# wwang2/CoarseGrainingVAE

Measured on AMD Instinct MI355X. Metric: train_step_frames_per_sec, higher is better.
Workload: dtype f32

## Files before the change

coarsegrainingvae_amd/_lib.py:

```python
from __future__ import annotations

import ctypes as C
import os
import re
import threading

import torch

from . import ktimer

_PKG = os.path.dirname(os.path.abspath(__file__))
LIB_PATH = os.environ.get("CGV_LIB") or os.path.join(_PKG, "libcgvae_hip.so")
HEADER_PATH = os.path.join(os.path.dirname(_PKG), "include", "cgvae_hip.h")

_lock = threading.Lock()
_lib = None

_p, _i, _f, _sz = C.c_void_p, C.c_int, C.c_float, C.c_size_t

PROTOTYPES = {
    "cgv_version": (_i, []),
    "cgv_last_error_string": (C.c_char_p, []),
    "cgv_timestamp": (_i, [_p, _p]),
    "cgv_timestamp_hz": (_i, []),
    "cgv_sustained_clock_probe": (_i, [_p, _p, _i, _i, _p]),
    "cgv_set_option": (_i, [_i, _i]),
    "cgv_get_option": (_i, [_i]),
    "cgv_reset_options": (_i, []),
    "cgv_rbf_supported": (_i, [_i]),
    "cgv_geom_stride": (_i, [_i]),
    "cgv_geom_unit_offset": (_i, [_i]),
    "cgv_radius_graph_count": (_i, [_p, _p, _i, _i, _f, _i, _p, _p, _p]),
    "cgv_radius_graph_emit": (_i, [_p, _p, _i, _i, _f, _i, _p, _p, _p]),
    "cgv_csr_workspace_bytes": (_sz, [_i]),
    "cgv_csr_build": (_i, [_p, _p, _i, _i, _i, _i, _p, _p, _p, _p, _p, _p, _p, _p, _p, _sz, _p]),
    "cgv_group_plan_workspace_bytes": (_sz, [_i]),
    "cgv_group_plan_build": (_i, [_p, _p, _p, _i, _i, _i, _i, _p, _p, _p, _p, _p, _sz, _p]),
    "cgv_group_plan_radix_workspace_bytes": (_sz, [_i]),
    "cgv_group_plan_build_radix": (_i, [_p, _p, _i, _i, _i, _i, _p, _p, _p, _p, _p, _sz, _p]),
    "cgv_geom_group_stride": (_i, [_i]),
    "cgv_geom_group_unit_offset": (_i, [_i]),
    "cgv_edge_geometry_grouped": (_i, [_p, _p, _p, _p, _p, _i, _i, _f, _p, _p, _p]),
    "cgv_edge_geometry": (_i, [_p, _p, _p, _p, _p, _p, _i, _i, _f, _p, _p, _p]),
    "cgv_plan_jobs_max": (_i, []),
    "cgv_plan_job_bytes": (_i, []),
    "cgv_plan_jobs_build": (_i, [_p, _i, _p]),
    "cgv_geom_jobs_max": (_i, []),
    "cgv_geom_job_bytes": (_i, []),
    "cgv_geom_jobs_build": (_i, [_p, _i, _p]),
    "cgv_segment_reduce": (_i, [_p, _p, _p, _i, _i, _i, _p, _p]),
    "cgv_embedding_rows": (_i, [_p, _p, _i, _i, _i, _i, _p, _p]),
    "cgv_embedding_rows2": (_i, [_p, _p, _i, _i, _i, _p, _p, _p, _i, _i, _i, _p, _i, _p]),
    "cgv_segment_reduce_pair": (_i, [_p, _p, _p, _i, _p, _p, _p, _p, _i, _p, _i, _p]),
    "cgv_segment_broadcast": (_i, [_p, _p, _p, _i, _i, _i, _p, _p]),
    "cgv_equi_msg_fwd": (_i, [_p, _p, _p, _p, _p, _p, _p, _p, _p, _i, _i, _i, _i, C.c_int64, C.c_int64, _p, _p, _p]),
    "cgv_equi_msg_grouped_supported": (_i, [_i, _i, _i]),
    "cgv_equi_msg_fwd_grouped": (_i, [_p] * 9 + [_i, _i, _i, _i, C.c_int64, C.c_int64, _p, _p, _p]),
    "cgv_equi_msg_bwd_workspace_bytes": (_sz, [_i, _i, _i]),
    "cgv_equi_msg_bwd": (_i, [_p] * 13 + [_i, _i, _i, C.c_int64, C.c_int64, _p, _sz, _p]),
    "cgv_pseudo_msg_fwd": (_i, [_p] * 14 + [_i, _i, _i, _i, _p]),
    "cgv_pseudo_msg_fwd_rows": (_i, [_p] * 15 + [_i, _i, _i, _i, C.c_int64, _p]),
    "cgv_pseudo_msg_bwd_workspace_bytes": (_sz, [_i, _i, _i]),
    "cgv_pseudo_msg_bwd": (_i, [_p] * 24 + [_i, _i, _i, _i, C.c_int64, _p, _sz, _p]),
    "cgv_pseudo_msg_bwd_deferred": (_i, [_p] * 22 + [_i, _i, _i, _i, C.c_int64, _p, _sz, _p, _p]),
    "cgv_update_rows_from_vec": (_i, [_p, _p, _i, _i, _p]),
    "cgv_tile_bwd_input_plan": (_i, [_i, _i, _i, _i, _p, _p]),
    "cgv_tile_linear_bwd_input_norm_stack": (_i, [_p, _p, _p, _i, _i, _i, _i, _p, _p, _p, _p, _p, _i, _i, _p]),
    "cgv_update_vec_from_rows": (_i, [_p, _p, _p, _i, _i, _p]),
    "cgv_update_norm_stack_fwd": (_i, [_p, _p, _p, _i, _i, _i, _p]),
# ... 204 lines not shown
    "cgv_cgae_resident_fits": (_i, [_i, _i, _i]),
    "cgv_cgae_workspace_bytes": (_sz, [_i, _i, _i, _i]),
    "cgv_cgae_steps": (_i, [_i] + [_p] * 7 + [_i, _p, C.c_int64, _i, _i, _i, _i, C.c_int64, _i, _f] + [C.c_double] * 4 +
                       [C.c_uint64, _p, _p, _p, _p, _sz, _p]),
    "cgv_cgae_noise": (_i, [C.c_uint64, C.c_int64, _i, _i, _i, _p, _p]),
    "cgv_newman_resident_fits": (_i, [_i, _i]),
    "cgv_newman_groups": (_i, [_i, _i]),
    "cgv_newman_workspace_bytes": (_sz, [_i, _i, _i, _i]),
    "cgv_newman_betweenness": (_i, [_p] * 4 + [_i] * 4 + [_p, _p, _sz, _p]),
    "cgv_newman_components": (_i, [_p] * 5 + [_i] * 4 + [_p, _p, _p, _sz, _p]),
    "cgv_newman_partition": (_i, [_p] * 8 + [_i] * 6 + [_p, _sz, _p]),
    "cgv_baseline_resident_fits": (_i, [_i, _i, _i, _i]),
    "cgv_baseline_workspace_bytes": (_sz, [_i] * 7),
    "cgv_baseline_steps": (_i, [_i, _i, _i] + [_p] * 4 + [_i, _p, C.c_int64] + [_i] * 5 + [_p, _p, _p, _i, C.c_int64, _i, _f] +
                           [C.c_double] * 4 + [_p, _p, _p, _sz, _p]),
    "cgv_baseline_loss_workspace_bytes": (_sz, [_i, _i, _i]),
    "cgv_baseline_loss": (_i, [_p, _p, _p, _i, _i, _i, _f, _p, _p, _p, _sz, _p]),
}


OPTIONS = {"msg_fwd_split": 0, "msg_bwd_split": 1, "csr_build": 2, "pseudo_chunks": 3, "wgrad_tiling": 4, "tile_fwd_lds_min": 5,
           "bwd_input_waves": 6, "pseudo_fwd": 7, "decoder_fat": 8, "decoder_wlds": 9, "skinny_rows": 10, "tile_fwd_bal": 11,
           "optim_one_launch": 12, "decoder_colsplit": 13, "decoder_nodesplit": 14, "bwd_input_split": 15, "msg_bwd_mfma": 16,
           "streamk": 17}


def set_option(name: str, value: int) -> None:
    call("cgv_set_option", OPTIONS[name], int(value))


def get_option(name: str) -> int:
    return int(load().cgv_get_option(OPTIONS[name]))


def reset_options() -> None:
    call("cgv_reset_options")


def header_symbols():
    text = open(HEADER_PATH).read()
    text = re.sub(r"/\*.*?\*/", "", text, flags=re.S)
    return sorted(set(re.findall(r"\b(cgv_[a-z0-9_]+)\s*\(", text)))


def load():
    global _lib
    if _lib is not None:
# ... 80 lines not shown
```

coarsegrainingvae_amd/csrc/api.cpp:

```cpp
#include <stdarg.h>
#include <string.h>
#include <atomic>
#include "cgv_common.h"

namespace cgv {
static thread_local char g_err[512] = "";
void set_error(const char* fmt, ...) {
  va_list ap;
  va_start(ap, fmt);
  vsnprintf(g_err, sizeof(g_err), fmt, ap);
  va_end(ap);
}

static const int g_opt_default[] = {
     -1,    -1,     0,
     0,     0,       448,
     0,   0,         1,
     1,      0,        1,
     0,  2,   1,
     -1,  -1,      0};
static_assert(sizeof(g_opt_default) == CGV_OPT_COUNT * sizeof(int), "one default per CGV_OPT_*");
static std::atomic<int> g_opt[CGV_OPT_COUNT];
static void reset_options() {
  for (int i = 0; i < CGV_OPT_COUNT; ++i) g_opt[i].store(g_opt_default[i], std::memory_order_relaxed);
}
static const bool g_opt_ready = (reset_options(), true);
int option(int id) { return g_opt[id].load(std::memory_order_relaxed); }
}

extern "C" {
int cgv_version(void) { return CGV_VERSION; }
int cgv_set_option(int option, int value) {
  CGV_REQUIRE(option >= 0 && option < CGV_OPT_COUNT, "unknown option");
  cgv::g_opt[option].store(value, std::memory_order_relaxed);
  return 0;
}
int cgv_get_option(int option) {
  if (option < 0 || option >= CGV_OPT_COUNT) return INT32_MIN;
  return cgv::g_opt[option].load(std::memory_order_relaxed);
}
int cgv_reset_options(void) {
  cgv::reset_options();
  return 0;
// ... 16 lines not shown
```

coarsegrainingvae_amd/csrc/batch_plans.hip:

```cpp
#include <cstring>
#include "cgv_common.h"

namespace cgv {

constexpr int PJ_MAX = 8;
struct PlanJob {
  const int64_t* key;
  const int64_t* other;
  const float* ids_f32;
  int* rowptr;
  int* eid;
  int* key_sorted;
  int* other_sorted;
  int* count;
  int* tmp;
  unsigned long long* spill;
  int stride, E, n_rows;
  int edge_begin, row_begin;
  int ids_is_key, pad, pad_to;
  int n_other;
};
struct PlanJobs { int n, total_edges, total_rows, pad; PlanJob job[PJ_MAX]; };

__device__ __forceinline__ int pj_ids(const PlanJob& p, int e) {
  const int t = (int)p.ids_f32[(int64_t)e * p.stride];
  return t == p.pad ? p.pad_to : t;
}
__device__ __forceinline__ int pj_key(const PlanJob& p, int e) {
  if (p.ids_f32 && p.ids_is_key) return pj_ids(p, e);
  return p.key ? (int)p.key[(int64_t)e * p.stride] : e;
}
__device__ __forceinline__ int pj_other(const PlanJob& p, int e) {
  if (p.ids_f32 && !p.ids_is_key) return pj_ids(p, e);
  return p.other ? (int)p.other[(int64_t)e * p.stride] : e;
}

__device__ __forceinline__ int pj_find_edge(const PlanJobs& J, int e) {
  int j = 0;
#pragma unroll
  for (int t = 1; t < PJ_MAX; ++t) if (t < J.n && J.job[t].edge_begin <= e) j = t;
  return j;
}

struct PjRun { int head_lane, len; bool head; };
__device__ __forceinline__ PjRun pj_run(int tag ) {
  const int lane = threadIdx.x & 63;
  const int prev = __shfl_up(tag, 1);
  const bool head = lane == 0 || tag != prev;
  const unsigned long long heads = __ballot(head);
  const unsigned long long below = heads & ((2ull << lane) - 1ull);
  const unsigned long long above = lane == 63 ? 0ull : heads & ~((2ull << lane) - 1ull);
  PjRun r;
  r.head = head;
  r.head_lane = 63 - __clzll((long long)below);
  const int end = above ? __ffsll((long long)above) - 1 : 64;
  r.len = end - r.head_lane;
  return r;
}

__global__ __launch_bounds__(256) void pj_count_k(PlanJobs J) {
  const int e = blockIdx.x * 256 + threadIdx.x;
  const bool active = e < J.total_edges;
  int* addr = nullptr;
  int tag = -1;
  if (active) {
    const int j = pj_find_edge(J, e);
    const PlanJob& p = J.job[j];
    const int r = pj_key(p, e - p.edge_begin);
    addr = p.count + r;
    tag = (j << 27) | r;
  }
  const PjRun run = pj_run(tag);
  if (active && run.head) atomicAdd(addr, run.len);
}

__global__ __launch_bounds__(1024) void pj_scan_k(PlanJobs J) {
  const PlanJob& p = J.job[blockIdx.x];
  const int* in = p.count;
  int* out = p.rowptr;
  const int n = p.n_rows;
  __shared__ int wave_tot[16];
  __shared__ int carry_s;
  const int tid = threadIdx.x, lane = tid & 63, w = tid >> 6;
  if (tid == 0) carry_s = 0;
  __syncthreads();
  for (int base = 0; base < n; base += 1024) {
    const int i = base + tid;
    const int x = (i < n) ? in[i] : 0;
    int incl = x;
    for (int d = 1; d < 64; d <<= 1) {
      const int y = __shfl_up(incl, d);
      if (lane >= d) incl += y;
    }
    if (lane == 63) wave_tot[w] = incl;
    __syncthreads();
    int wave_off = 0;
    for (int k = 0; k < w; ++k) wave_off += wave_tot[k];
// ... 98 lines not shown
  __syncthreads();
  for (int t = tid; t < L; t += 128) {
    const unsigned long long mine = k[t];
    const unsigned partner = (unsigned)(mine >> 32);
    int pos = hist[partner];
    if (hist[partner + 1] - pos > 1)
      for (int u = 0; u < L; ++u) pos += (k[u] >> 32) == partner && k[u] < mine;
    p.eid[beg + pos] = (int)(unsigned)(mine & 0xffffffffull);
    p.other_sorted[beg + pos] = (int)partner;
    p.key_sorted[beg + pos] = r;
  }
}

__global__ __launch_bounds__(128) void pj_row_sort_k(PlanJobs J) {
  __shared__ unsigned long long keys[PJ_LDS_KEYS];
  __shared__ int hist[PJ_HIST_MAX + 1];
  int j = 0;
#pragma unroll
  for (int t = 1; t < PJ_MAX; ++t) if (t < J.n && J.job[t].row_begin <= (int)blockIdx.x) j = t;
  const PlanJob& p = J.job[j];
  const int r = blockIdx.x - p.row_begin;
  const int beg = p.rowptr[r], L = p.rowptr[r + 1] - beg;
  if (L <= 0) return;
  if (L <= PJ_LDS_KEYS && L >= PJ_COUNT_FROM && p.n_other > 0 && p.n_other <= PJ_HIST_MAX) pj_count_row(keys, hist, p, r, beg, L);
  else if (L <= PJ_LDS_KEYS) pj_rank_row(keys, p, r, beg, L);
  else pj_rank_row(p.spill + beg, p, r, beg, L);
}

constexpr int GJ_MAX = 12;
struct GeomJob {
  const float* pos_dst; const float* pos_src;
  const int* dst; const int* src;
  const int2* meta;
  const float* coef;
  float* geom;
  float cutoff;
  int E, R, GS, edge_begin;
};
struct GeomJobs { int n, total_edges; GeomJob job[GJ_MAX]; };

constexpr int GJ_REC_MAX = 28;
__global__ __launch_bounds__(256) void gj_records_k(GeomJobs J) {
  __shared__ __attribute__((aligned(16))) float recs[256][GJ_REC_MAX];
  const int e_first = blockIdx.x * 256;
  const int e_raw = e_first + threadIdx.x;
  const bool valid = e_raw < J.total_edges;
// ... 43 lines not shown
    g[R + 5] = __int_as_float(m.y);
    for (int k = R + 6; k < GS; ++k) g[k] = 0.0f;
  } else {
    const int U = geom_unit_offset(R);
    for (int k = R + 1; k < U; ++k) g[k] = 0.0f;
    g[U + 0] = ux; g[U + 1] = uy; g[U + 2] = uz;
    g[U + 3] = ux; g[U + 4] = uy; g[U + 5] = uz;
    for (int k = U + 6; k < GS; ++k) g[k] = 0.0f;
  }
  if (!one_job) {
    if (valid)
      for (int k4 = 0; k4 < GS / 4; ++k4) dst4[k4] = reinterpret_cast<const float4*>(g)[k4];
    return;
  }
  __syncthreads();
  const int n_rec = min(256, J.total_edges - e_first), GS4 = GS >> 2;
  float4* out4 = reinterpret_cast<float4*>(q.geom + (size_t)(e_first - q.edge_begin) * GS);
  for (int idx = threadIdx.x; idx < n_rec * GS4; idx += 256) {
    const int r = idx / GS4, k4 = idx - r * GS4;
    out4[idx] = reinterpret_cast<const float4*>(recs[r])[k4];
  }
}

__global__ __launch_bounds__(256) void batch_rows_k(const float4* __restrict__ src_a, float4* __restrict__ dst_a,
                                                    float* __restrict__ xyz_a, int n_a, const float4* __restrict__ src_b,
                                                    float4* __restrict__ dst_b, float* __restrict__ xyz_b, int n_b) {
  int i = blockIdx.x * 256 + threadIdx.x;
  const float4* src = src_a; float4* dst = dst_a; float* xyz = xyz_a;
  if (i >= n_a) { i -= n_a; src = src_b; dst = dst_b; xyz = xyz_b; if (i >= n_b) return; }
  const float4 r = src[i];
  dst[i] = r;
  xyz[3 * (size_t)i + 0] = r.y; xyz[3 * (size_t)i + 1] = r.z; xyz[3 * (size_t)i + 2] = r.w;
}

}

extern "C" {

int cgv_batch_load_rows(const float* src_atoms, float* dst_atoms, float* xyz_atoms, int n_atoms, const float* src_beads,
                        float* dst_beads, float* xyz_beads, int n_beads, void* stream) {
  CGV_REQUIRE(src_atoms && dst_atoms && xyz_atoms && src_beads && dst_beads && xyz_beads && n_atoms >= 0 && n_beads >= 0, "bad argument");
  const int n = n_atoms + n_beads;
  if (n == 0) return 0;
  hipLaunchKernelGGL(cgv::batch_rows_k, dim3((n + 255) / 256), dim3(256), 0, (hipStream_t)stream,
                     reinterpret_cast<const float4*>(src_atoms), reinterpret_cast<float4*>(dst_atoms), xyz_atoms, n_atoms,
                     reinterpret_cast<const float4*>(src_beads), reinterpret_cast<float4*>(dst_beads), xyz_beads, n_beads);
  return cgv::check_launch("cgv_batch_load_rows");
}

int cgv_plan_jobs_max(void) { return cgv::PJ_MAX; }
int cgv_plan_job_bytes(void) { return (int)sizeof(cgv::PlanJob); }
int cgv_geom_jobs_max(void) { return cgv::GJ_MAX; }
int cgv_geom_job_bytes(void) { return (int)sizeof(cgv::GeomJob); }

int cgv_plan_jobs_build(const void* jobs_host, int n_jobs, void* stream) {
  CGV_REQUIRE(jobs_host && n_jobs >= 1 && n_jobs <= cgv::PJ_MAX, "bad job table");
  cgv::PlanJobs J;
  std::memset(static_cast<void*>(&J), 0, sizeof(J));
  std::memcpy(static_cast<void*>(J.job), jobs_host, sizeof(cgv::PlanJob) * (size_t)n_jobs);
  J.n = n_jobs;
  int e = 0, r = 0;
  for (int j = 0; j < n_jobs; ++j) {
    cgv::PlanJob& p = J.job[j];
    CGV_REQUIRE(p.E >= 0 && p.n_rows >= 0 && p.n_rows < (1 << 27) && p.stride >= 1 && p.rowptr && p.count, "bad job");
    CGV_REQUIRE(p.E == 0 || (p.eid && p.key_sorted && p.other_sorted && p.tmp && p.spill), "null edge array");
    CGV_REQUIRE(p.n_other >= 0, "bad partner range");
    p.edge_begin = e; p.row_begin = r;
    e += p.E; r += p.n_rows;
  }
  J.total_edges = e; J.total_rows = r;
  hipStream_t st = (hipStream_t)stream;
  if (e > 0) hipLaunchKernelGGL(cgv::pj_count_k, dim3((e + 255) / 256), dim3(256), 0, st, J);
  hipLaunchKernelGGL(cgv::pj_scan_k, dim3(n_jobs), dim3(1024), 0, st, J);
  if (e > 0) {
    hipLaunchKernelGGL(cgv::pj_drop_k, dim3((e + 255) / 256), dim3(256), 0, st, J);
    if (r > 0) hipLaunchKernelGGL(cgv::pj_row_sort_k, dim3(r), dim3(128), 0, st, J);
  }
  return cgv::check_launch("cgv_plan_jobs_build");
}

int cgv_geom_jobs_build(const void* jobs_host, int n_jobs, void* stream) {
  CGV_REQUIRE(jobs_host && n_jobs >= 1 && n_jobs <= cgv::GJ_MAX, "bad job table");
  cgv::GeomJobs J;
  std::memset(static_cast<void*>(&J), 0, sizeof(J));
  std::memcpy(static_cast<void*>(J.job), jobs_host, sizeof(cgv::GeomJob) * (size_t)n_jobs);
  J.n = n_jobs;
  int e = 0;
  for (int j = 0; j < n_jobs; ++j) {
    cgv::GeomJob& q = J.job[j];
    CGV_REQUIRE(q.E >= 0 && q.R > 0 && cgv_rbf_supported(q.R) && q.coef && q.geom && q.pos_dst && q.pos_src && q.dst && q.src, "bad job");
    q.GS = q.meta ? cgv::geom_group_stride(q.R) : cgv::geom_stride(q.R);
    q.edge_begin = e;
    e += q.E;
  }
  J.total_edges = e;
  if (e == 0) return 0;
  hipLaunchKernelGGL(cgv::gj_records_k, dim3((e + 255) / 256), dim3(256), 0, (hipStream_t)stream, J);
  return cgv::check_launch("cgv_geom_jobs_build");
}

}
// ... 1 lines not shown
```

coarsegrainingvae_amd/data.py:

```python
from __future__ import annotations

from typing import Dict, List, Optional

import numpy as np
import torch
from torch.utils.data import Dataset as TorchDataset

from .graph import BatchGraph, radius_graph

_KEYS = ("nxyz", "CG_nxyz", "num_atoms", "num_CGs", "CG_mapping", "bond_edge_list")


def batch_to(batch, device):
    return {k: (v.to(device) if hasattr(v, "to") else v) for k, v in batch.items()}


def CG_collate(dicts: List[Dict[str, torch.Tensor]]) -> Dict[str, torch.Tensor]:
    atoms0 = np.cumsum([0] + [int(d["num_atoms"]) for d in dicts])[:-1]
    beads0 = np.cumsum([0] + [int(d["num_CGs"]) for d in dicts])[:-1]
    atom_keys, bead_keys = ("nbr_list", "bond_edge_list"), ("CG_mapping", "CG_nbr_list")
    batch = {}
    for key, first in dicts[0].items():
        vals = [d[key] for d in dicts]
        if key in atom_keys:
# ... 69 lines not shown
    cg_nbrs = staged(make_directed(src["CG_nbr_list"])[0]).to(dev, non_blocking=True)
    g.update(dst["nxyz"][:, 1:], dst["CG_nxyz"][:, 1:], atom_nbrs, cg_nbrs, directed=True)
    dst["nbr_list"], dst["CG_nbr_list"] = src["nbr_list"], src["CG_nbr_list"]
    return True


def _copy_prepared_into(dst, src, g, sg) -> bool:
    accepted = dst.setdefault("_accepted", {})
    hit = accepted.get(id(src))
    if hit is None or hit[0] is not src:
        ok = all(k in src and tuple(src[k].shape) == tuple(dst[k].shape) for k in _STATIC_KEYS)
        ok = ok and src["nxyz"].device == dst["nxyz"].device
        ok = ok and bool(torch.equal(src["bond_edge_list"], dst["bond_edge_list"]))
        ok = ok and bool(torch.equal(sg.mapping, g.mapping))
        ok = ok and bool(torch.equal(src["num_atoms"], dst["num_atoms"])) and bool(torch.equal(src["num_CGs"], dst["num_CGs"]))
        accepted[id(src)] = hit = (src, ok)
    if not hit[1]:
        return False
    if sg.atom_nbrs.shape[0] > g.atom.capacity or sg.cg_nbrs.shape[0] > g.cg.capacity:
        return False
    rows = (src["nxyz"], dst["nxyz"], src["CG_nxyz"], dst["CG_nxyz"])
    if all(t.dtype == torch.float32 and t.is_contiguous() and t.dim() == 2 and t.shape[1] == 4 for t in rows) \
            and g.xyz.is_contiguous() and g.cg_xyz.is_contiguous():
        from . import _lib
        _lib.call("cgv_batch_load_rows", _lib.ptr(rows[0]), _lib.ptr(rows[1]), _lib.ptr(g.xyz), int(rows[0].shape[0]),
                  _lib.ptr(rows[2]), _lib.ptr(rows[3]), _lib.ptr(g.cg_xyz), int(rows[2].shape[0]), _lib.stream_ptr())
        g.update(g.xyz, g.cg_xyz, sg.atom_nbrs, sg.cg_nbrs, directed=True)
    else:
        for k in _MOVING_KEYS:
            dst[k].copy_(src[k], non_blocking=True)
        g.update(dst["nxyz"][:, 1:], dst["CG_nxyz"][:, 1:], sg.atom_nbrs, sg.cg_nbrs, directed=True)
    dst["nbr_list"], dst["CG_nbr_list"] = src["nbr_list"], src["CG_nbr_list"]
    return True


class CGDataset(TorchDataset):

    def __init__(self, props, check_props=True):
        self.props = props

    def __len__(self):
        return len(self.props["nxyz"])

    def __getitem__(self, idx):
        return {key: val[idx] for key, val in self.props.items()}

    def generate_neighbor_list(self, atom_cutoff, cg_cutoff, device="cuda", undirected=True, use_bond=False):
        if use_bond:
            self.props["nbr_list"] = self.props["bond_edge_list"]
        else:
# ... 145 lines not shown
```

coarsegrainingvae_amd/graph.py:

```python
from __future__ import annotations

from typing import Optional, Tuple

import ctypes as C

import numpy as np
import torch

from . import _lib

_I32 = torch.int32


class PlanJob(C.Structure):
    _fields_ = [("key", C.c_void_p), ("other", C.c_void_p), ("ids_f32", C.c_void_p), ("rowptr", C.c_void_p), ("eid", C.c_void_p),
                ("key_sorted", C.c_void_p), ("other_sorted", C.c_void_p), ("count", C.c_void_p), ("tmp", C.c_void_p),
                ("spill", C.c_void_p), ("stride", C.c_int), ("E", C.c_int), ("n_rows", C.c_int), ("edge_begin", C.c_int),
                ("row_begin", C.c_int), ("ids_is_key", C.c_int), ("pad", C.c_int), ("pad_to", C.c_int), ("n_other", C.c_int)]


class GeomJob(C.Structure):
    _fields_ = [("pos_dst", C.c_void_p), ("pos_src", C.c_void_p), ("dst", C.c_void_p), ("src", C.c_void_p),
                ("meta", C.c_void_p), ("coef", C.c_void_p), ("geom", C.c_void_p), ("cutoff", C.c_float), ("E", C.c_int),
                ("R", C.c_int), ("GS", C.c_int), ("edge_begin", C.c_int)]


def cutoff_threshold_sq(cutoff: float, strict: bool = False) -> float:
    c = np.float32(cutoff)
    if not np.isfinite(c) or c < 0:
        raise ValueError("cutoff must be a finite non-negative number")
    if strict and c == 0:
        raise ValueError("the strict threshold needs a positive cutoff (no s has sqrt(s) < 0)")
    guess = np.float32(c) * np.float32(c)
    bits = int(np.array(guess, dtype=np.float32).view(np.uint32))
    lo, hi = max(bits - 64, 0), bits + 64

    pattern = np.arange(lo, hi + 1, dtype=np.uint32).view(np.float32).copy()
    roots = torch.sqrt(torch.from_numpy(pattern))
    window = ((roots < torch.tensor(c)) if strict else (roots <= torch.tensor(c))).tolist()
    if not window[0] or window[-1]:
        raise RuntimeError("cutoff threshold search window does not bracket the cutoff")
# ... 86 lines not shown
            return
        lib = _lib.load()
        if radix:
            ws_bytes = int(lib.cgv_group_plan_radix_workspace_bytes(self.n_edges))
            ws = torch.empty(ws_bytes, dtype=torch.uint8, device=self.device)
            _lib.call("cgv_group_plan_build_radix", _lib.ptr(self.dst_d), _lib.ptr(self.src_d), self.n_edges, self.n_dst,
                      self.n_src, self.group_rb, _lib.ptr(self.dst_g), _lib.ptr(self.src_g), _lib.ptr(self.pos_g),
                      _lib.ptr(self.meta_g), _lib.ptr(ws), ws_bytes, _lib.stream_ptr())
            return
        ws_bytes = int(lib.cgv_group_plan_workspace_bytes(self.capacity))
        if self._grp_ws is None or self._grp_ws.numel() < ws_bytes:
            self._grp_ws = torch.empty(ws_bytes, dtype=torch.uint8, device=self.device)
        ws = self._grp_ws
        _lib.call("cgv_group_plan_build", _lib.ptr(self.rowptr_d), _lib.ptr(self.dst_d), _lib.ptr(self.src_d), self.n_edges,
                  self.n_dst, self.n_src, self.group_rb, _lib.ptr(self.dst_g), _lib.ptr(self.src_g), _lib.ptr(self.pos_g),
                  _lib.ptr(self.meta_g), _lib.ptr(ws), ws_bytes, _lib.stream_ptr())

    def view_jobs(self, dst: torch.Tensor, src: Optional[torch.Tensor], stride: int, n_edges: int):
        if n_edges > self.capacity:
            raise ValueError(f"{n_edges} edges exceed the plan's capacity of {self.capacity}")
        if self._job_ws is None:
            E, dev = self.capacity, self.device
            mk = lambda n, dt=_I32: torch.zeros(n, dtype=dt, device=dev)
            self._job_ws = [(mk(rows + 1), mk(E), mk(E, torch.int64)) for rows in (self.n_dst, self.n_src)]
        self.n_edges = int(n_edges)
        self._job_keep = (dst, src)
        d_ptr, s_ptr = dst.data_ptr(), (src.data_ptr() if src is not None else None)
        (cd, td, sd), (cs, ts, ss) = self._job_ws
        jd = PlanJob(d_ptr, s_ptr, None, self.rowptr_d.data_ptr(), self.eid_d.data_ptr(), self.dst_d.data_ptr(), self.src_d.data_ptr(),
                     cd.data_ptr(), td.data_ptr(), sd.data_ptr(), stride, self.n_edges, self.n_dst, 0, 0, 0, 0, 0,
                     self.n_src if src is not None else 0)
        js = PlanJob(s_ptr, d_ptr, None, self.rowptr_s.data_ptr(), self.eid_s.data_ptr(), self.src_s.data_ptr(), self.dst_s.data_ptr(),
                     cs.data_ptr(), ts.data_ptr(), ss.data_ptr(), stride, self.n_edges, self.n_src, 0, 0, 0, 0, 0, self.n_dst)
        return [jd, js]

    def nbrs_jobs(self, nbrs: torch.Tensor):
        nbrs = nbrs.long().contiguous()
        if nbrs.shape[0] == 0:
            dummy = torch.zeros(2, dtype=torch.int64, device=self.device)
            return self.view_jobs(dummy, dummy[1:], 2, 0)
        flat = nbrs.view(-1)
        return self.view_jobs(flat, flat[1:], 2, nbrs.shape[0])

    def mapping_jobs(self, mapping: torch.Tensor):
        mapping = mapping.long().contiguous()
        if mapping.shape[0] != self.n_edges:
            raise ValueError("a mapping plan keeps its length")
        return self.view_jobs(mapping, None, 1, mapping.shape[0])

    def type_id_jobs(self, ids_f32: torch.Tensor, pad, pad_to: int):
        if ids_f32.dtype != torch.float32 or ids_f32.dim() != 1 or ids_f32.shape[0] != self.n_edges:
            raise ValueError("type ids must be a float32 column of the plan's length")
        jobs = self.view_jobs(ids_f32, None, int(ids_f32.stride(0)), ids_f32.shape[0])
        for k, job in enumerate(jobs):
            job.key, job.other, job.ids_f32, job.n_other = None, None, ids_f32.data_ptr(), 0
            job.ids_is_key = 1 if k == 0 else 0
# ... 159 lines not shown

    def _positions(self, which: str):
        if which == "atom":
            return self.atom, self.xyz, self.xyz
        if which == "cg":
            return self.cg, self.cg_xyz, self.cg_xyz
        if which == "a2b":
            return self.a2b, self.cg_xyz, self.xyz
        raise KeyError(which)

    def fits(self, xyz, cg_xyz, mapping, nbr_list, cg_nbr_list) -> bool:
        if self.dir_mp:
            return False
        if not (tuple(xyz.shape) == tuple(self.xyz.shape) and tuple(cg_xyz.shape) == tuple(self.cg_xyz.shape)
                and 2 * nbr_list.shape[0] <= self.atom.capacity and 2 * cg_nbr_list.shape[0] <= self.cg.capacity
                and tuple(mapping.shape) == tuple(self.mapping.shape)):
            return False
        if mapping.is_cuda:
            return bool(torch.equal(mapping.long(), self.mapping))
        if self.mapping_cpu is None:
            self.mapping_cpu = self.mapping.cpu()
        return bool(torch.equal(mapping.long(), self.mapping_cpu))

    def update(self, xyz, cg_xyz, nbr_list, cg_nbr_list, directed: bool = False):
        if self.dir_mp:
            raise RuntimeError("a dir_mp bundle is not re-planned in place: prepare the new batch with prepare_batch(dir_mp=True)")
        dev = self.xyz.device
        if xyz.data_ptr() != self.xyz.data_ptr():
            self.xyz.copy_(xyz.detach().float(), non_blocking=True)
        if cg_xyz.data_ptr() != self.cg_xyz.data_ptr():
            self.cg_xyz.copy_(cg_xyz.detach().float(), non_blocking=True)
        if directed:
            self.atom_nbrs, self.cg_nbrs = nbr_list, cg_nbr_list
        else:
            self.atom_nbrs = make_directed(nbr_list)[0].to(dev)
            self.cg_nbrs = make_directed(cg_nbr_list)[0].to(dev)
        if self._update_by_jobs():
            return
        self.atom.rebuild_from_nbrs(self.atom_nbrs)
        self.cg.rebuild_from_nbrs(self.cg_nbrs)
        for (which, _r, _c), g in self._geom.items():
            plan, pd, ps = self._positions(which)
            g.rebuild(plan, pos_dst=pd, pos_src=ps)
        for (_which, n_types, pad), (plan, idx) in self._embed.items():
            ids = idx.long()
            if pad is not None:
                ids = torch.where(ids == pad, torch.full_like(ids, n_types), ids)
            plan.rebuild_from_mapping(ids)

    def _update_by_jobs(self) -> bool:
        lib = _lib.load()
        if self.xyz.device.type != "cuda" or lib.cgv_plan_job_bytes() != C.sizeof(PlanJob) or lib.cgv_geom_job_bytes() != C.sizeof(GeomJob):
            return False
        plan_jobs = self.atom.nbrs_jobs(self.atom_nbrs) + self.cg.nbrs_jobs(self.cg_nbrs)
        for (_which, n_types, pad), (plan, idx) in self._embed.items():
            if idx.dtype == torch.float32 and idx.dim() == 1:
                plan_jobs += plan.type_id_jobs(idx, pad, n_types)
            else:
                ids = idx.long()
                if pad is not None:
                    ids = torch.where(ids == pad, torch.full_like(ids, n_types), ids)
                plan_jobs += plan.mapping_jobs(ids)
        geom_jobs = []
        for (which, _r, _c), g in self._geom.items():
            plan, pd, ps = self._positions(which)
            geom_jobs += g.jobs(plan, pd, ps)
        if len(plan_jobs) > lib.cgv_plan_jobs_max() or len(geom_jobs) > lib.cgv_geom_jobs_max():
            return False
        st = _lib.stream_ptr()
        table = (PlanJob * len(plan_jobs))(*plan_jobs)
        _lib.call("cgv_plan_jobs_build", C.addressof(table), len(plan_jobs), st)
        if self.atom.group_rb:
            self.atom._build_groups()
        if geom_jobs:
            gt = (GeomJob * len(geom_jobs))(*geom_jobs)
            _lib.call("cgv_geom_jobs_build", C.addressof(gt), len(geom_jobs), st)
        return True

    def embed_plan(self, which: str, idx: torch.Tensor, module) -> EdgePlan:
        key = (which, int(module.weight.shape[0]), module.padding_idx)
        hit = self._embed.get(key)
        if hit is None:
            from .ops import embedding_plan
            hit = self._embed[key] = (embedding_plan(idx, module.weight.shape[0], module.padding_idx), idx)
        return hit[0]

    def geometry(self, which: str, n_rbf: int, cutoff: float) -> EdgeGeometry:
        key = (which, int(n_rbf), float(cutoff))
        g = self._geom.get(key)
        if g is None:
            if which == "atom":
                g = EdgeGeometry(self.atom, n_rbf, cutoff, pos_dst=self.xyz, pos_src=self.xyz)
            elif which == "cg":
                g = EdgeGeometry(self.cg, n_rbf, cutoff, pos_dst=self.cg_xyz, pos_src=self.cg_xyz)
# ... 7 lines not shown
```

include/cgvae_hip.h:

```cpp
#ifndef CGVAE_HIP_H
#define CGVAE_HIP_H

#include <stddef.h>
#include <stdint.h>

#ifdef __cplusplus
extern "C" {
#endif

#define CGV_VERSION 101

#define CGV_E_BADARG (-1)
#define CGV_E_UNSUPPORTED (-2)
#define CGV_E_WORKSPACE (-3)

int cgv_version(void);
const char* cgv_last_error_string(void);

enum {
  CGV_OPT_MSG_FWD_SPLIT = 0,
  CGV_OPT_MSG_BWD_SPLIT = 1,
  CGV_OPT_CSR_BUILD = 2,
  CGV_OPT_PSEUDO_CHUNKS = 3,
  CGV_OPT_WGRAD_TILING = 4,
  CGV_OPT_TILE_FWD_LDS_MIN = 5,
  CGV_OPT_BWD_INPUT_WAVES = 6,
  CGV_OPT_PSEUDO_FWD = 7,
  CGV_OPT_DECODER_FAT = 8,
  CGV_OPT_DECODER_WLDS = 9,
  CGV_OPT_SKINNY_ROWS = 10,
  CGV_OPT_TILE_FWD_BAL = 11,
  CGV_OPT_OPTIM_ONE_LAUNCH = 12,
  CGV_OPT_DECODER_COLSPLIT = 13,
  CGV_OPT_DECODER_NODESPLIT = 14,
  CGV_OPT_BWD_INPUT_SPLIT = 15,
  CGV_OPT_MSG_BWD_MFMA = 16,
  CGV_OPT_STREAMK = 17,
  CGV_OPT_COUNT = 18
};
int cgv_timestamp(uint64_t* slot , void* stream);
int cgv_timestamp_hz(void);
int cgv_sustained_clock_probe(uint64_t* out , float* sink , int blocks, int iters, void* stream);
int cgv_set_option(int option, int value);
int cgv_get_option(int option);
int cgv_reset_options(void);

int cgv_rbf_supported(int n_rbf);
int cgv_geom_stride(int n_rbf);
int cgv_geom_unit_offset(int n_rbf);

int cgv_radius_graph_count(const float* xyz , const int32_t* frame_ptr ,
                           int n_frames, int n_nodes, float s_star, int undirected,
                           int32_t* counts , int32_t* offsets , void* stream);
int cgv_radius_graph_emit(const float* xyz, const int32_t* frame_ptr, int n_frames, int n_nodes, float s_star,
                          int undirected, const int32_t* offsets , int64_t* nbr_out ,
                          void* stream);

size_t cgv_csr_workspace_bytes(int n_edges);
int cgv_csr_build(const int64_t* dst, const int64_t* src, int stride, int n_edges, int n_dst, int n_src,
                  int32_t* rowptr_d, int32_t* eid_d, int32_t* dst_d, int32_t* src_d,
                  int32_t* rowptr_s, int32_t* eid_s, int32_t* dst_s, int32_t* src_s,
// ... 58 lines not shown
                             float* dv , int n_dst, int n_feat, int n_rbf, int rb, int64_t n_rows,
                             int64_t n_edges , const float* s_res , const float* v_res ,
                             void* stream);
size_t cgv_equi_msg_bwd_workspace_bytes(int n_src, int n_feat, int n_rbf);
int cgv_equi_msg_bwd(const float* phi, const float* v, const float* geom_s, const int32_t* rowptr_s,
                     const int32_t* dst_s, const float* Wd, const float* bd, const float* gs ,
                     const float* gv , float* g_phi, float* g_v, float* gWd, float* gbd,
                     int n_src, int n_feat, int n_rbf, int64_t n_edges_hint, int64_t n_rows_hint, void* workspace,
                     size_t workspace_bytes, void* stream);
int cgv_equi_msg_bwd_deferred(const float* phi, const float* v, const float* geom_s, const int32_t* rowptr_s,
                              const int32_t* dst_s, const float* Wd, const float* bd, const float* gs, const float* gv,
                              float* g_phi, float* g_v, int n_src, int n_feat, int n_rbf, int64_t n_edges_hint,
                              int64_t n_rows_hint, void* workspace, size_t workspace_bytes, int* n_chunks, int* k_live,
                              void* stream);
int cgv_filter_reduce_jobs_max(void);
int cgv_filter_reduce_job_bytes(void);
int cgv_filter_reduce_jobs(const void* jobs_host, int n_jobs, void* stream);

int cgv_batch_load_rows(const float* src_atoms, float* dst_atoms, float* xyz_atoms, int n_atoms, const float* src_beads,
                        float* dst_beads, float* xyz_beads, int n_beads, void* stream);
int cgv_plan_jobs_max(void);
int cgv_plan_job_bytes(void);
int cgv_plan_jobs_build(const void* jobs_host, int n_jobs, void* stream);
int cgv_geom_jobs_max(void);
int cgv_geom_job_bytes(void);
int cgv_geom_jobs_build(const void* jobs_host, int n_jobs, void* stream);

int cgv_pseudo_msg_fwd(const float* phi , const float* s, const float* sbar, const float* v,
                       const float* vbar, const float* geom_d, const int32_t* rowptr_d, const int32_t* src_d,
                       const float* Wd , const float* bd , float* dh, float* dhbar, float* dv,
                       float* dvbar, int n_nodes, int n_feat, int n_rbf, int residual, void* stream);
int cgv_pseudo_msg_fwd_rows(const float* phi, const float* s, const float* sbar, const float* v, const float* vbar,
                            const float* geom_d, const int32_t* rowptr_d, const int32_t* src_d, const float* Wd,
                            const float* bd, float* dh, float* dhbar, float* dv, float* dvbar, float* dv_rows,
                            int n_nodes, int n_feat, int n_rbf, int residual, int64_t n_edges_hint ,
                            void* stream);
size_t cgv_pseudo_msg_bwd_workspace_bytes(int n_nodes, int n_feat, int n_rbf);
int cgv_pseudo_msg_bwd(const float* phi, const float* s, const float* sbar, const float* v, const float* vbar,
                       const float* geom_d, const int32_t* rowptr_d, const int32_t* src_d,
                       const float* geom_s, const int32_t* rowptr_s, const int32_t* dst_s,
                       const float* Wd, const float* bd,
                       const float* gh, const float* ghbar, const float* gv, const float* gvbar,
                       float* g_phi , float* g_s, float* g_sbar, float* g_v, float* g_vbar,
                       float* gWd , float* gbd , int n_nodes, int n_feat, int n_rbf,
                       int residual, int64_t n_edges_hint , void* workspace,
                       size_t workspace_bytes, void* stream);
// ... 420 lines not shown
```

Measured before the change: 1287.

## Fuse batch row load with plan count, and scan with edge drop

Adds a fused plan-building path, on by default. The batch row copy now runs in the same launch as the per-row edge counting, and the prefix scan is merged into the edge-drop kernel, with each block redoing the small scan in LDS. Count buffers are doubled so drop offsets can be taken with atomics, and the row-sort kernel clears them for the next build. The aim is to cut kernel launches and inter-kernel dependencies in the per-step graph re-plan. The cost is redundant scan work per block, and the fused path only applies when rows and edge counts stay under fixed limits.

```diff
diff --git a/coarsegrainingvae_amd/_lib.py b/coarsegrainingvae_amd/_lib.py
--- a/coarsegrainingvae_amd/_lib.py
+++ b/coarsegrainingvae_amd/_lib.py
@@ -45,6 +45,11 @@
     "cgv_plan_jobs_max": (_i, []),
     "cgv_plan_job_bytes": (_i, []),
     "cgv_plan_jobs_build": (_i, [_p, _i, _p]),
+    "cgv_batch_plans_build": (_i, [_p, _i, _p, _p, _p, _i, _p, _p, _p, _i, _p]),
+    "cgv_plan_fused_fits": (_i, [_i, _i]),
+    "cgv_plan_fused_max_rows": (_i, []),
+    "cgv_plan_fused_max_edges": (_i, []),
+    "cgv_plan_path_count": (C.c_longlong, [_i]),
     "cgv_geom_jobs_max": (_i, []),
     "cgv_geom_job_bytes": (_i, []),
     "cgv_geom_jobs_build": (_i, [_p, _i, _p]),
@@ -295,7 +300,7 @@
 OPTIONS = {"msg_fwd_split": 0, "msg_bwd_split": 1, "csr_build": 2, "pseudo_chunks": 3, "wgrad_tiling": 4, "tile_fwd_lds_min": 5,
            "bwd_input_waves": 6, "pseudo_fwd": 7, "decoder_fat": 8, "decoder_wlds": 9, "skinny_rows": 10, "tile_fwd_bal": 11,
            "optim_one_launch": 12, "decoder_colsplit": 13, "decoder_nodesplit": 14, "bwd_input_split": 15, "msg_bwd_mfma": 16,
-           "streamk": 17}
+           "streamk": 17, "plan_fused": 18}
 
 
 def set_option(name: str, value: int) -> None:
diff --git a/coarsegrainingvae_amd/csrc/api.cpp b/coarsegrainingvae_amd/csrc/api.cpp
--- a/coarsegrainingvae_amd/csrc/api.cpp
+++ b/coarsegrainingvae_amd/csrc/api.cpp
@@ -18,7 +18,8 @@
      0,   0,         1,
      1,      0,        1,
      0,  2,   1,
-     -1,  -1,      0};
+     -1,  -1,      0,
+     1};
 static_assert(sizeof(g_opt_default) == CGV_OPT_COUNT * sizeof(int), "one default per CGV_OPT_*");
 static std::atomic<int> g_opt[CGV_OPT_COUNT];
 static void reset_options() {
diff --git a/coarsegrainingvae_amd/csrc/batch_plans.hip b/coarsegrainingvae_amd/csrc/batch_plans.hip
--- a/coarsegrainingvae_amd/csrc/batch_plans.hip
+++ b/coarsegrainingvae_amd/csrc/batch_plans.hip
@@ -1,3 +1,4 @@
+#include <atomic>
 #include <cstring>
 #include "cgv_common.h"
 
@@ -19,8 +20,9 @@
   int edge_begin, row_begin;
   int ids_is_key, pad, pad_to;
   int n_other;
+  int cap;
 };
-struct PlanJobs { int n, total_edges, total_rows, pad; PlanJob job[PJ_MAX]; };
+struct PlanJobs { int n, total_edges, total_rows, fused; PlanJob job[PJ_MAX]; };
 
 __device__ __forceinline__ int pj_ids(const PlanJob& p, int e) {
   const int t = (int)p.ids_f32[(int64_t)e * p.stride];
@@ -58,8 +60,7 @@
   return r;
 }
 
-__global__ __launch_bounds__(256) void pj_count_k(PlanJobs J) {
-  const int e = blockIdx.x * 256 + threadIdx.x;
+__device__ __forceinline__ void pj_count_edge(const PlanJobs& J, int e) {
   const bool active = e < J.total_edges;
   int* addr = nullptr;
   int tag = -1;
@@ -73,6 +74,7 @@
   const PjRun run = pj_run(tag);
   if (active && run.head) atomicAdd(addr, run.len);
 }
+__global__ __launch_bounds__(256) void pj_count_k(PlanJobs J) { pj_count_edge(J, blockIdx.x * 256 + threadIdx.x); }
 
 __global__ __launch_bounds__(1024) void pj_scan_k(PlanJobs J) {
   const PlanJob& p = J.job[blockIdx.x];
@@ -217,6 +219,7 @@
   const int r = blockIdx.x - p.row_begin;
   const int beg = p.rowptr[r], L = p.rowptr[r + 1] - beg;
   if (L <= 0) return;
+  if (J.fused && threadIdx.x == 0) { p.count[r] = 0; p.count[p.n_rows + 1 + r] = 0; }
   if (L <= PJ_LDS_KEYS && L >= PJ_COUNT_FROM && p.n_other > 0 && p.n_other <= PJ_HIST_MAX) pj_count_row(keys, hist, p, r, beg, L);
   else if (L <= PJ_LDS_KEYS) pj_rank_row(keys, p, r, beg, L);
   else pj_rank_row(p.spill + beg, p, r, beg, L);
@@ -306,20 +309,76 @@
   }
 }
 
-__global__ __launch_bounds__(256) void batch_rows_k(const float4* __restrict__ src_a, float4* __restrict__ dst_a,
-                                                    float* __restrict__ xyz_a, int n_a, const float4* __restrict__ src_b,
-                                                    float4* __restrict__ dst_b, float* __restrict__ xyz_b, int n_b) {
-  int i = blockIdx.x * 256 + threadIdx.x;
-  const float4* src = src_a; float4* dst = dst_a; float* xyz = xyz_a;
-  if (i >= n_a) { i -= n_a; src = src_b; dst = dst_b; xyz = xyz_b; if (i >= n_b) return; }
+struct RowsLoad { const float4* src_a; float4* dst_a; float* xyz_a; int n_a; const float4* src_b; float4* dst_b; float* xyz_b; int n_b; };
+__device__ __forceinline__ void batch_rows_at(const RowsLoad& L, int i) {
+  const float4* src = L.src_a; float4* dst = L.dst_a; float* xyz = L.xyz_a;
+  if (i >= L.n_a) { i -= L.n_a; src = L.src_b; dst = L.dst_b; xyz = L.xyz_b; if (i >= L.n_b) return; }
   const float4 r = src[i];
   dst[i] = r;
   xyz[3 * (size_t)i + 0] = r.y; xyz[3 * (size_t)i + 1] = r.z; xyz[3 * (size_t)i + 2] = r.w;
 }
+__global__ __launch_bounds__(256) void batch_rows_k(RowsLoad L) { batch_rows_at(L, blockIdx.x * 256 + threadIdx.x); }
+
+constexpr int PJ_FUSED_ROWS_MAX = 1024, PJ_FUSED_EDGES_MAX = 65536;
+struct PjBlocks { int begin[PJ_MAX + 1]; };
+
+__global__ __launch_bounds__(256) void pj_count_rows_k(PlanJobs J, RowsLoad L, int count_blocks) {
+  if ((int)blockIdx.x < count_blocks) pj_count_edge(J, blockIdx.x * 256 + threadIdx.x);
+  else batch_rows_at(L, ((int)blockIdx.x - count_blocks) * 256 + threadIdx.x);
+}
+
+__global__ __launch_bounds__(256) void pj_scan_drop_k(PlanJobs J, PjBlocks B) {
+  __shared__ int row_s[PJ_FUSED_ROWS_MAX + 1];
+  __shared__ int wave_tot[4];
+  int j = 0;
+#pragma unroll
+  for (int t = 1; t < PJ_MAX; ++t) if (t < J.n && B.begin[t] <= (int)blockIdx.x) j = t;
+  const PlanJob& p = J.job[j];
+  const int n = p.n_rows, tid = threadIdx.x, lane = tid & 63;
+  const int C = (n + 255) / 256, b0 = min(tid * C, n), b1 = min(b0 + C, n);
+  int sum = 0;
+  for (int b = b0; b < b1; ++b) sum += p.count[b];
+  int incl = sum;
+#pragma unroll
+  for (int d = 1; d < 64; d <<= 1) {
+    const int up = __shfl_up(incl, d);
+    if (lane >= d) incl += up;
+  }
+  if (lane == 63) wave_tot[tid >> 6] = incl;
+  __syncthreads();
+  int run_sum = incl - sum;
+  for (int w = 0; w < (tid >> 6); ++w) run_sum += wave_tot[w];
+  for (int b = b0; b < b1; ++b) { row_s[b] = run_sum; run_sum += p.count[b]; }
+  if (tid == 255) row_s[n] = run_sum;
+  __syncthreads();
+  const int lb = (int)blockIdx.x - B.begin[j];
+  if (lb == 0)
+    for (int b = tid; b <= n; b += 256) p.rowptr[b] = row_s[b];
+  const int le = lb * 256 + tid;
+  const bool active = le < p.E;
+  int r = 0, tag = -1;
+  if (active) {
+    r = min(max(pj_key(p, le), 0), n - 1);
+    tag = r;
+  }
+  const PjRun run = pj_run(tag);
+  int base = 0;
+  if (active && run.head) base = atomicAdd(p.count + (n + 1) + r, run.len);
+  base = __shfl(base, run.head_lane);
+  if (active) p.tmp[row_s[r] + base + (lane - run.head_lane)] = le;
+}
 
 }
 
 extern "C" {
+
+static cgv::RowsLoad rows_load(const float* src_atoms, float* dst_atoms, float* xyz_atoms, int n_atoms, const float* src_beads,
+                               float* dst_beads, float* xyz_beads, int n_beads) {
+  cgv::RowsLoad L;
+  L.src_a = reinterpret_cast<const float4*>(src_atoms); L.dst_a = reinterpret_cast<float4*>(dst_atoms); L.xyz_a = xyz_atoms; L.n_a = n_atoms;
+  L.src_b = reinterpret_cast<const float4*>(src_beads); L.dst_b = reinterpret_cast<float4*>(dst_beads); L.xyz_b = xyz_beads; L.n_b = n_beads;
+  return L;
+}
 
 int cgv_batch_load_rows(const float* src_atoms, float* dst_atoms, float* xyz_atoms, int n_atoms, const float* src_beads,
                         float* dst_beads, float* xyz_beads, int n_beads, void* stream) {
@@ -327,8 +386,7 @@
   const int n = n_atoms + n_beads;
   if (n == 0) return 0;
   hipLaunchKernelGGL(cgv::batch_rows_k, dim3((n + 255) / 256), dim3(256), 0, (hipStream_t)stream,
-                     reinterpret_cast<const float4*>(src_atoms), reinterpret_cast<float4*>(dst_atoms), xyz_atoms, n_atoms,
-                     reinterpret_cast<const float4*>(src_beads), reinterpret_cast<float4*>(dst_beads), xyz_beads, n_beads);
+                     rows_load(src_atoms, dst_atoms, xyz_atoms, n_atoms, src_beads, dst_beads, xyz_beads, n_beads));
   return cgv::check_launch("cgv_batch_load_rows");
 }
 
@@ -336,10 +394,15 @@
 int cgv_plan_job_bytes(void) { return (int)sizeof(cgv::PlanJob); }
 int cgv_geom_jobs_max(void) { return cgv::GJ_MAX; }
 int cgv_geom_job_bytes(void) { return (int)sizeof(cgv::GeomJob); }
-
-int cgv_plan_jobs_build(const void* jobs_host, int n_jobs, void* stream) {
+int cgv_plan_fused_max_rows(void) { return cgv::PJ_FUSED_ROWS_MAX; }
+int cgv_plan_fused_max_edges(void) { return cgv::PJ_FUSED_EDGES_MAX; }
+
+static std::atomic<long long> g_plan_builds[2];
+long long cgv_plan_path_count(int fused) { return g_plan_builds[fused ? 1 : 0].load(std::memory_order_relaxed); }
+
+static int plan_jobs_table(const char* who, const void* jobs_host, int n_jobs, cgv::PlanJobs& J) {
+  (void)who;
   CGV_REQUIRE(jobs_host && n_jobs >= 1 && n_jobs <= cgv::PJ_MAX, "bad job table");
-  cgv::PlanJobs J;
   std::memset(static_cast<void*>(&J), 0, sizeof(J));
   std::memcpy(static_cast<void*>(J.job), jobs_host, sizeof(cgv::PlanJob) * (size_t)n_jobs);
   J.n = n_jobs;
@@ -348,19 +411,80 @@
     cgv::PlanJob& p = J.job[j];
     CGV_REQUIRE(p.E >= 0 && p.n_rows >= 0 && p.n_rows < (1 << 27) && p.stride >= 1 && p.rowptr && p.count, "bad job");
     CGV_REQUIRE(p.E == 0 || (p.eid && p.key_sorted && p.other_sorted && p.tmp && p.spill), "null edge array");
-    CGV_REQUIRE(p.n_other >= 0, "bad partner range");
+    CGV_REQUIRE(p.n_other >= 0 && p.cap >= 0, "bad partner range / capacity");
     p.edge_begin = e; p.row_begin = r;
     e += p.E; r += p.n_rows;
   }
   J.total_edges = e; J.total_rows = r;
-  hipStream_t st = (hipStream_t)stream;
+  return 0;
+}
+
+static void plan_jobs_launch(const cgv::PlanJobs& J, hipStream_t st) {
+  const int e = J.total_edges, r = J.total_rows;
   if (e > 0) hipLaunchKernelGGL(cgv::pj_count_k, dim3((e + 255) / 256), dim3(256), 0, st, J);
-  hipLaunchKernelGGL(cgv::pj_scan_k, dim3(n_jobs), dim3(1024), 0, st, J);
+  hipLaunchKernelGGL(cgv::pj_scan_k, dim3(J.n), dim3(1024), 0, st, J);
   if (e > 0) {
     hipLaunchKernelGGL(cgv::pj_drop_k, dim3((e + 255) / 256), dim3(256), 0, st, J);
     if (r > 0) hipLaunchKernelGGL(cgv::pj_row_sort_k, dim3(r), dim3(128), 0, st, J);
   }
+  g_plan_builds[0].fetch_add(1, std::memory_order_relaxed);
+}
+
+int cgv_plan_jobs_build(const void* jobs_host, int n_jobs, void* stream) {
+  cgv::PlanJobs J;
+  if (int rc = plan_jobs_table("cgv_plan_jobs_build", jobs_host, n_jobs, J)) return rc;
+  plan_jobs_launch(J, (hipStream_t)stream);
   return cgv::check_launch("cgv_plan_jobs_build");
+}
+
+int cgv_plan_fused_fits(int n_rows, int edge_capacity) {
+  return n_rows >= 1 && n_rows <= cgv::PJ_FUSED_ROWS_MAX && edge_capacity >= 1 && edge_capacity <= cgv::PJ_FUSED_EDGES_MAX;
+}
+
+int cgv_batch_plans_build(const void* jobs_host, int n_jobs, const float* src_atoms, float* dst_atoms, float* xyz_atoms,
+                          int n_atoms, const float* src_beads, float* dst_beads, float* xyz_beads, int n_beads, void* stream) {
+  cgv::PlanJobs J;
+  if (int rc = plan_jobs_table("cgv_batch_plans_build", jobs_host, n_jobs, J)) return rc;
+  const bool rows = src_atoms != nullptr;
+  CGV_REQUIRE(!rows || (dst_atoms && xyz_atoms && src_beads && dst_beads && xyz_beads && n_atoms >= 0 && n_beads >= 0), "bad argument");
+  hipStream_t st = (hipStream_t)stream;
+  bool fused = cgv::option(CGV_OPT_PLAN_FUSED) != 0;
+  for (int j = 0; j < n_jobs; ++j) fused = fused && J.job[j].cap >= J.job[j].E && cgv_plan_fused_fits(J.job[j].n_rows, J.job[j].cap);
+  if (!fused) {
+    if (rows) {
+      int rc = cgv_batch_load_rows(src_atoms, dst_atoms, xyz_atoms, n_atoms, src_beads, dst_beads, xyz_beads, n_beads, stream);
+      if (rc) return rc;
+    }
+    plan_jobs_launch(J, st);
+    return cgv::check_launch("cgv_batch_plans_build");
+  }
+  J.fused = 1;
+  cgv::PjBlocks B;
+  int blocks = 0;
+  for (int j = 0; j < cgv::PJ_MAX + 1; ++j) {
+    B.begin[j] = blocks;
+    if (j < n_jobs) blocks += J.job[j].E > 0 ? (J.job[j].E + 255) / 256 : 1;
+  }
+  cgv::PlanJobs Jc = J;
+  cgv::RowsLoad L;
+  std::memset(static_cast<void*>(&L), 0, sizeof(L));
+  int row_blocks = 0;
+  if (rows) {
+    L = rows_load(src_atoms, dst_atoms, xyz_atoms, n_atoms, src_beads, dst_beads, xyz_beads, n_beads);
+    row_blocks = (n_atoms + n_beads + 255) / 256;
+    for (int j = 0; j < n_jobs; ++j) {
+      const float* ids = Jc.job[j].ids_f32;
+      if (ids && ids >= dst_atoms && ids < dst_atoms + 4 * (size_t)n_atoms) Jc.job[j].ids_f32 = src_atoms + (ids - dst_atoms);
+      else if (ids && ids >= dst_beads && ids < dst_beads + 4 * (size_t)n_beads) Jc.job[j].ids_f32 = src_beads + (ids - dst_beads);
+    }
+  }
+  const int e = J.total_edges, count_blocks = (e + 255) / 256;
+  if (count_blocks + row_blocks > 0)
+    hipLaunchKernelGGL(cgv::pj_count_rows_k, dim3(count_blocks + row_blocks), dim3(256), 0, st, Jc, L, count_blocks);
+  hipLaunchKernelGGL(cgv::pj_scan_drop_k, dim3(blocks), dim3(256), 0, st, J, B);
+  if (e > 0 && J.total_rows > 0) hipLaunchKernelGGL(cgv::pj_row_sort_k, dim3(J.total_rows), dim3(128), 0, st, J);
+  g_plan_builds[1].fetch_add(1, std::memory_order_relaxed);
+  return cgv::check_launch("cgv_batch_plans_build");
 }
 
 int cgv_geom_jobs_build(const void* jobs_host, int n_jobs, void* stream) {
diff --git a/coarsegrainingvae_amd/data.py b/coarsegrainingvae_amd/data.py
--- a/coarsegrainingvae_amd/data.py
+++ b/coarsegrainingvae_amd/data.py
@@ -115,10 +115,7 @@
     rows = (src["nxyz"], dst["nxyz"], src["CG_nxyz"], dst["CG_nxyz"])
     if all(t.dtype == torch.float32 and t.is_contiguous() and t.dim() == 2 and t.shape[1] == 4 for t in rows) \
             and g.xyz.is_contiguous() and g.cg_xyz.is_contiguous():
-        from . import _lib
-        _lib.call("cgv_batch_load_rows", _lib.ptr(rows[0]), _lib.ptr(rows[1]), _lib.ptr(g.xyz), int(rows[0].shape[0]),
-                  _lib.ptr(rows[2]), _lib.ptr(rows[3]), _lib.ptr(g.cg_xyz), int(rows[2].shape[0]), _lib.stream_ptr())
-        g.update(g.xyz, g.cg_xyz, sg.atom_nbrs, sg.cg_nbrs, directed=True)
+        g.update(g.xyz, g.cg_xyz, sg.atom_nbrs, sg.cg_nbrs, directed=True, load_rows=rows)
     else:
         for k in _MOVING_KEYS:
             dst[k].copy_(src[k], non_blocking=True)
diff --git a/coarsegrainingvae_amd/graph.py b/coarsegrainingvae_amd/graph.py
--- a/coarsegrainingvae_amd/graph.py
+++ b/coarsegrainingvae_amd/graph.py
@@ -16,7 +16,8 @@
     _fields_ = [("key", C.c_void_p), ("other", C.c_void_p), ("ids_f32", C.c_void_p), ("rowptr", C.c_void_p), ("eid", C.c_void_p),
                 ("key_sorted", C.c_void_p), ("other_sorted", C.c_void_p), ("count", C.c_void_p), ("tmp", C.c_void_p),
                 ("spill", C.c_void_p), ("stride", C.c_int), ("E", C.c_int), ("n_rows", C.c_int), ("edge_begin", C.c_int),
-                ("row_begin", C.c_int), ("ids_is_key", C.c_int), ("pad", C.c_int), ("pad_to", C.c_int), ("n_other", C.c_int)]
+                ("row_begin", C.c_int), ("ids_is_key", C.c_int), ("pad", C.c_int), ("pad_to", C.c_int), ("n_other", C.c_int),
+                ("cap", C.c_int)]
 
 
 class GeomJob(C.Structure):
@@ -149,7 +150,7 @@
         if self._job_ws is None:
             E, dev = self.capacity, self.device
             mk = lambda n, dt=_I32: torch.zeros(n, dtype=dt, device=dev)
-            self._job_ws = [(mk(rows + 1), mk(E), mk(E, torch.int64)) for rows in (self.n_dst, self.n_src)]
+            self._job_ws = [(mk(2 * (rows + 1)), mk(E), mk(E, torch.int64)) for rows in (self.n_dst, self.n_src)]
         self.n_edges = int(n_edges)
         self._job_keep = (dst, src)
         d_ptr, s_ptr = dst.data_ptr(), (src.data_ptr() if src is not None else None)
@@ -159,6 +160,7 @@
                      self.n_src if src is not None else 0)
         js = PlanJob(s_ptr, d_ptr, None, self.rowptr_s.data_ptr(), self.eid_s.data_ptr(), self.src_s.data_ptr(), self.dst_s.data_ptr(),
                      cs.data_ptr(), ts.data_ptr(), ss.data_ptr(), stride, self.n_edges, self.n_src, 0, 0, 0, 0, 0, self.n_dst)
+        jd.cap = js.cap = max(self.capacity, 1)
         return [jd, js]
 
     def nbrs_jobs(self, nbrs: torch.Tensor):
@@ -364,7 +366,7 @@
             self.mapping_cpu = self.mapping.cpu()
         return bool(torch.equal(mapping.long(), self.mapping_cpu))
 
-    def update(self, xyz, cg_xyz, nbr_list, cg_nbr_list, directed: bool = False):
+    def update(self, xyz, cg_xyz, nbr_list, cg_nbr_list, directed: bool = False, load_rows=None):
         if self.dir_mp:
             raise RuntimeError("a dir_mp bundle is not re-planned in place: prepare the new batch with prepare_batch(dir_mp=True)")
         dev = self.xyz.device
@@ -377,8 +379,10 @@
         else:
             self.atom_nbrs = make_directed(nbr_list)[0].to(dev)
             self.cg_nbrs = make_directed(cg_nbr_list)[0].to(dev)
-        if self._update_by_jobs():
+        if self._update_by_jobs(load_rows):
             return
+        if load_rows is not None:
+            self._load_rows(load_rows)
         self.atom.rebuild_from_nbrs(self.atom_nbrs)
         self.cg.rebuild_from_nbrs(self.cg_nbrs)
         for (which, _r, _c), g in self._geom.items():
@@ -390,10 +394,22 @@
                 ids = torch.where(ids == pad, torch.full_like(ids, n_types), ids)
             plan.rebuild_from_mapping(ids)
 
-    def _update_by_jobs(self) -> bool:
+    def _load_rows(self, rows):
+        _lib.call("cgv_batch_load_rows", _lib.ptr(rows[0]), _lib.ptr(rows[1]), _lib.ptr(self.xyz), int(rows[0].shape[0]),
+                  _lib.ptr(rows[2]), _lib.ptr(rows[3]), _lib.ptr(self.cg_xyz), int(rows[2].shape[0]), _lib.stream_ptr())
+
+    def _update_by_jobs(self, load_rows=None) -> bool:
         lib = _lib.load()
         if self.xyz.device.type != "cuda" or lib.cgv_plan_job_bytes() != C.sizeof(PlanJob) or lib.cgv_geom_job_bytes() != C.sizeof(GeomJob):
             return False
+        n_geom = sum(3 if (g.geom_g is not None and self._positions(which)[0].group_rb) else 2
+                     for (which, _r, _c), g in self._geom.items())
+        if 4 + 2 * len(self._embed) > lib.cgv_plan_jobs_max() or n_geom > lib.cgv_geom_jobs_max():
+            return False
+        ids_in_kernel = all(idx.dtype == torch.float32 and idx.dim() == 1 for _plan, idx in self._embed.values())
+        if load_rows is not None and not ids_in_kernel:
+            self._load_rows(load_rows)
+            load_rows = None
         plan_jobs = self.atom.nbrs_jobs(self.atom_nbrs) + self.cg.nbrs_jobs(self.cg_nbrs)
         for (_which, n_types, pad), (plan, idx) in self._embed.items():
             if idx.dtype == torch.float32 and idx.dim() == 1:
@@ -407,11 +423,14 @@
         for (which, _r, _c), g in self._geom.items():
             plan, pd, ps = self._positions(which)
             geom_jobs += g.jobs(plan, pd, ps)
-        if len(plan_jobs) > lib.cgv_plan_jobs_max() or len(geom_jobs) > lib.cgv_geom_jobs_max():
-            return False
         st = _lib.stream_ptr()
         table = (PlanJob * len(plan_jobs))(*plan_jobs)
-        _lib.call("cgv_plan_jobs_build", C.addressof(table), len(plan_jobs), st)
+        rows = load_rows if load_rows is not None else (None, None, None, None)
+        _lib.call("cgv_batch_plans_build", C.addressof(table), len(plan_jobs),
+                  _lib.ptr(rows[0]), _lib.ptr(rows[1]), _lib.ptr(self.xyz) if load_rows is not None else None,
+                  int(rows[0].shape[0]) if load_rows is not None else 0,
+                  _lib.ptr(rows[2]), _lib.ptr(rows[3]), _lib.ptr(self.cg_xyz) if load_rows is not None else None,
+                  int(rows[2].shape[0]) if load_rows is not None else 0, st)
         if self.atom.group_rb:
             self.atom._build_groups()
         if geom_jobs:
diff --git a/include/cgvae_hip.h b/include/cgvae_hip.h
--- a/include/cgvae_hip.h
+++ b/include/cgvae_hip.h
@@ -36,7 +36,8 @@
   CGV_OPT_BWD_INPUT_SPLIT = 15,
   CGV_OPT_MSG_BWD_MFMA = 16,
   CGV_OPT_STREAMK = 17,
-  CGV_OPT_COUNT = 18
+  CGV_OPT_PLAN_FUSED = 18,
+  CGV_OPT_COUNT = 19
 };
 int cgv_timestamp(uint64_t* slot , void* stream);
 int cgv_timestamp_hz(void);
@@ -141,6 +142,12 @@
 int cgv_plan_jobs_max(void);
 int cgv_plan_job_bytes(void);
 int cgv_plan_jobs_build(const void* jobs_host, int n_jobs, void* stream);
+int cgv_batch_plans_build(const void* jobs_host, int n_jobs, const float* src_atoms, float* dst_atoms, float* xyz_atoms,
+                          int n_atoms, const float* src_beads, float* dst_beads, float* xyz_beads, int n_beads, void* stream);
+int cgv_plan_fused_fits(int n_rows, int edge_capacity);
+int cgv_plan_fused_max_rows(void);
+int cgv_plan_fused_max_edges(void);
+long long cgv_plan_path_count(int fused);
 int cgv_geom_jobs_max(void);
 int cgv_geom_job_bytes(void);
 int cgv_geom_jobs_build(const void* jobs_host, int n_jobs, void* stream);
```

Result: no change. 1290, median of 6 (+0.2%).
